# hzyu17/GaussianVI

Hardware: AMD Instinct MI355X
Metric: sigma-point psi-evals/sec + NGD iters/sec, 1024-factor d=12 p=5 chain (higher is better)
Workload: dtype f64; 1 GPU; c3: T=1025 states, n=6; 1 step = 1 device-resident NGD iteration; restart every 30; factor_sets_columns=[K factors, d, GH degree p, N sigma points], factor_set_kinds=1024 x quadratic-prior d=12 p=5 (N=17217); 1025 x fixed-prior d=6 p=5 (N=1433), kernel_variant=6, chunks_per_factor=4, fused_pass=True, one_launch_factor_stage=False, mirror_pairs=False, fuse_trial=2

## Files before the change

### gaussianvi_amd/csrc/gvi_hip.hip

```cpp
#include "../../include/gvi_hip.h"

#include <hip/hip_runtime.h>
#include <hip/hip_ext.h>
#include <dlfcn.h>

#include <algorithm>
#include <chrono>
#include <cmath>
#include <cstdio>
#include <cstdlib>
#include <cstring>
#include <memory>
#include <map>
#include <set>
#include <string>
#include <thread>
#include <type_traits>
#include <vector>

#include "host_linalg.hpp"
#include "kernels_bt.hpp"
#include "chain_launch.hpp"
#include "kernels_factor.hpp"
#include "kernels_orbit.hpp"
// ... 491 lines not shown
  const int nb0 = nbx0 * a0.nchunk, nb1 = nbx1 * a1.nchunk;
  const int grid = std::max(nb0, nb1);
  if (full)
    hipExtLaunchKernelGGL((moments_orbit_pair_kernel<M, SMAX, true, false, WAVES>), dim3(grid), dim3(256), (uint32_t)lds, st, e0, e1, 0,
                          a0, a1, nbx0, nb0, nbx1);
  else
    hipExtLaunchKernelGGL((moments_orbit_pair_kernel<M, SMAX, false, false, WAVES>), dim3(grid), dim3(256), (uint32_t)lds, st, e0, e1, 0,
                          a0, a1, nbx0, nb0, nbx1);
}

void launch_orbit_pair(const OrbitArgs& a0, const OrbitArgs& a1, int m, int smax, bool full, hipStream_t st, hipEvent_t e0, hipEvent_t e1) {
  const size_t lds = (size_t)4 * std::max(orbit_lds_doubles(a0.d, m, a0.copies), orbit_lds_doubles(a1.d, m, a1.copies)) * 8;
  with_orbit_instance(m, smax, [&]<int M, int SMAX, int WAVES, bool PAIR>(OrbitInst<M, SMAX, WAVES, PAIR>) {
    if constexpr (PAIR) launch_orbit_pair_t<M, SMAX, WAVES>(a0, a1, full, lds, st, e0, e1);
  });
}

inline std::atomic<long long>* fused_launches() { static std::atomic<long long> c[3]; return c; }

inline std::atomic<long long>& block3_launches() { static std::atomic<long long> c; return c; }

template <int M, int SMAX, int WAVES, int D0, int D1>
gvi_status launch_fused_t(gvi_ctx* c, const FusedArgs& A, unsigned grid, size_t lds, int dmax, int copies, int items, hipEvent_t e0, hipEvent_t e1) {
  if (lds > 64 * 1024) GVICK(allow_lds(c, (const void*)factor_fused_kernel<M, SMAX, WAVES, D0, D1>, (int)lds));
#ifdef GVI_FUSED_TIMING
  const int dbg = getenv("GVI_FUSED_DBG") ? atoi(getenv("GVI_FUSED_DBG")) : 0;
  static unsigned long long* stamps = nullptr;
  static int nprint = 0;
  if ((dbg & 8) && !stamps) { if (hipMalloc(&stamps, 1120 * 8) != hipSuccess) stamps = nullptr; else (void)hipMemset(stamps, 0, 1120 * 8); }
#else
  const int dbg = 0;
  unsigned long long* stamps = nullptr;
#endif
  hipExtLaunchKernelGGL((factor_fused_kernel<M, SMAX, WAVES, D0, D1>), dim3(grid), dim3(256), (uint32_t)lds, c->stream, e0, e1, 0, A, dmax, copies, items,
                        (dbg & 8) ? stamps : (unsigned long long*)nullptr);
  ++fused_launches()[M == 2 ? 2 : (SMAX <= 4 ? 0 : 1)];
#ifdef GVI_FUSED_TIMING
  if ((dbg & 8) && stamps && ++nprint > 200 && nprint <= 202) {
    unsigned long long h[1120];
    (void)hipStreamSynchronize(c->stream);
    (void)hipMemcpy(h, stamps, sizeof(h), hipMemcpyDeviceToHost);
    for (int blk = 0; blk < 8; ++blk)
      for (int w = 0; w < 4; ++w)
        for (int it = 0; it < 2; ++it) {
          const unsigned long long* ws = h + 352 + ((blk * 4 + w) * 2 + it) * 12;
          fprintf(stderr, "[walk stamps] block %4d wave %d item %d: shader cycles prologue %llu | s=1 %llu (%llu tiles) | s=2 %llu (%llu) | s=3 %llu (%llu) | s=4 %llu (%llu) | reduction %llu\n",
                  blk * 146, w, it, ws[0], ws[1], ws[7], ws[2], ws[8], ws[3], ws[9], ws[4], ws[10], ws[5]);
        }
    for (int w = 0; w < 4; ++w) {
      fprintf(stderr, "[prep stamps] block 0 wave %d, us after the wave's start: prologue [arguments warm | first scalars | barrier] %.2f %.2f %.2f; gather [entry | loads back | stores issued] %.2f %.2f %.2f; products [Sigma row loaded | Cholesky | L^-1 | LDS | Lam + stores | H, u0]:",
              w, (double)(long long)(h[256 + 16 * w + 11] - h[8 * w]) * 0.01, (double)(long long)(h[256 + 16 * w + 12] - h[8 * w]) * 0.01,
              (double)(long long)(h[256 + 16 * w + 13] - h[8 * w]) * 0.01, (double)(long long)(h[256 + 16 * w + 8] - h[8 * w]) * 0.01, (double)(long long)(h[256 + 16 * w + 9] - h[8 * w]) * 0.01, (double)(long long)(h[256 + 16 * w + 10] - h[8 * w]) * 0.01);
      for (int i = 0; i < 6; ++i) fprintf(stderr, " %.2f", (double)(long long)(h[256 + 16 * w + i] - h[8 * w]) * 0.01);
      fprintf(stderr, "\n");
    }
    unsigned long long t0 = ~0ull;
    for (int blk = 0; blk < 8; ++blk) if (h[blk * 32] && h[blk * 32] < t0) t0 = h[blk * 32];
    for (int blk = 0; blk < 8; ++blk)
      for (int w = 0; w < 4; ++w) {
        const unsigned hw = (unsigned)h[320 + blk * 4 + w], xcc = (unsigned)(h[320 + blk * 4 + w] >> 32);
        fprintf(stderr, "[fused stamps] block %4d wave %d (xcc %u se %u cu %2u simd %u slot %2u; absolute, us after the first start):", blk * 146, w,
                xcc & 15, (hw >> 13) & 7, (hw >> 8) & 15, (hw >> 4) & 3, hw & 15);
        for (int i = 0; i < 8; ++i) fprintf(stderr, " %.2f", h[blk * 32 + w * 8 + i] ? (double)(long long)(h[blk * 32 + w * 8 + i] - t0) * 0.01 : -1.0);
        fprintf(stderr, "\n");
      }
  }
#endif
  return GVI_OK;
}

gvi_status launch_prep(gvi_ctx* c, const FactorDev& f, const double* mu, const double* Sigma, hipStream_t st) {
  const int d = f.d, dp = d + (d & 1);
  const size_t lds = (size_t)(4 * d * d + 2 * dp + 3 * d) * 8 + (size_t)dp * 4 + 16;
  if (d <= 8) hipLaunchKernelGGL(prep_kernel<1>, dim3(f.K), dim3(64), lds, st, f, mu, Sigma);
  else if (d <= 16) hipLaunchKernelGGL(prep_kernel<4>, dim3(f.K), dim3(64), lds, st, f, mu, Sigma);
  else if (d <= 32) hipLaunchKernelGGL(prep_kernel<16>, dim3(f.K), dim3(64), lds, st, f, mu, Sigma);
  else return fail(c, GVI_ERR_UNSUPPORTED, "factor dimension > 32");
  return GVI_OK;
}

gvi_status run_prep(gvi_ctx* c, FactorSet& s, const double* mu, const double* Sigma, int slot = -1,
                    hipStream_t st = nullptr) {
  if (!st) st = c->stream;
  if (slot >= 0 && s.prep_slot == slot) return GVI_OK;
  s.prep_slot = slot;
  if (s.K == 0) return GVI_OK;
  GVICK(launch_prep(c, s.dev(c->opt), mu, Sigma, st));
  HIPCK(c, hipGetLastError());
  return GVI_OK;
}

template <int KIND>
gvi_status launch_orbit_psi_t(gvi_ctx* c, const OrbitPsiArgs& a, bool full, dim3 grid, size_t lds, hipStream_t st) {
  if (full) {
    if (lds > 64 * 1024) GVICK(allow_lds(c, (const void*)moments_orbit_psi_kernel<KIND, true>, (int)lds));
    hipLaunchKernelGGL((moments_orbit_psi_kernel<KIND, true>), grid, dim3(256), lds, st, a);
  } else {
    hipLaunchKernelGGL((moments_orbit_psi_kernel<KIND, false>), grid, dim3(256), lds, st, a);
  }
  return GVI_OK;
}

struct MomPlan {
  Route route = Route::Empty;
  int full = 0;
  int nchunk = 1;
// ... 1480 lines not shown
      HIPCK(ctx, hipGetLastError());
      record_plan(s0, P[0], true);
      record_plan(s1, P[1], true);
      return prof_close(ctx, b);
    }
    case Fuse::SregPair:
    case Fuse::ScostPair: {
      FactorSet &s0 = *ctx->sets[0], &s1 = *ctx->sets[1];
      const MomArgs &a0 = P[0].a, &a1 = P[1].a;
      const int nbx0 = (int)P[0].grid.x, nbx1 = (int)P[1].grid.x;
      const int nb0 = nbx0 * (int)P[0].grid.y, nb1 = nbx1 * (int)P[1].grid.y;
      GVICK(prof_open(ctx, s0, 0, full != 0, true, ctx->stream, &b));
      if (full && P[0].pipe && P[1].pipe)
        hipLaunchKernelGGL((moments_sreg_pair_kernel<12, 6, 6, 6, true, true>), dim3(std::max(nb0, nb1)), dim3(256), 0, ctx->stream,
                           a0, a1, nbx0, nb0, nbx1);
      else if (full)
        hipLaunchKernelGGL((moments_sreg_pair_kernel<12, 6, 6, 6, true>), dim3(nb0 + nb1), dim3(256), 0, ctx->stream, a0, a1, nbx0, nb0, nbx1);
      else
        hipLaunchKernelGGL((moments_scost_pair_kernel<12, 6, 6, 6, 2>), dim3(nb0 + nb1), dim3(256), 0, ctx->stream, a0, a1, nbx0, nb0, nbx1);
      HIPCK(ctx, hipGetLastError());
      record_plan(s0, P[0], true);
      record_plan(s1, P[1], true);
      return prof_close(ctx, b);
    }
    case Fuse::Planar3: {
      int nbx[3], nb[3];
      for (int q = 0; q < 3; ++q) {
        nbx[q] = (ctx->sets[q]->K + 3) / 4;
        nb[q] = nbx[q] * P[q].nchunk;
      }
      GVICK(prof_open(ctx, *ctx->sets[1], 0, full != 0, true, ctx->stream, &b));
      if (full)
        hipLaunchKernelGGL((moments_planar3_kernel<true>), dim3(nb[0] + nb[1] + nb[2]), dim3(256), 0, ctx->stream, P[0].a, P[1].a, P[2].a,
                           nbx[0], nb[0], nbx[1], nb[1], nbx[2], P[0].pipe ? 1 : 0);
      else
        hipLaunchKernelGGL((moments_planar3_kernel<false>), dim3(nb[0] + nb[1] + nb[2]), dim3(256), 0, ctx->stream, P[0].a, P[1].a, P[2].a,
                           nbx[0], nb[0], nbx[1], nb[1], nbx[2], 0);
      HIPCK(ctx, hipGetLastError());
      for (int q = 0; q < 3; ++q) record_plan(*ctx->sets[q], P[q], false);
      return prof_close(ctx, b);
    }
    case Fuse::None:
      break;
  }
  for (int i = 0; i < ns; ++i) GVICK(launch_single(ctx, *ctx->sets[i], P[i], ctx->stream));
  return GVI_OK;
}

static gvi_status ngd_fused_full(gvi_ctx* ctx, int slot, int publish_slot, const PassPlan& pp) {
  constexpr int fused_chunks = 4;
  FusedArgs A{};
  A.nsets = (int)ctx->sets.size();
  A.koff[0] = 0;
  int dmax = 0, copies = 1;
  const FusedKey key = fused_key(A.nsets, pp.F);
  A.nblk = fused_nblk(pp.F[0].K, A.nsets > 1 ? pp.F[1].K : 0, FUSED_MAX_ITEMS);
  for (int si = 0; si < A.nsets; ++si) {
    FactorSet& s = *ctx->sets[si];
    FusedSet& F = A.s[si];
    s.prep_slot = -1;
    F.f = s.dev(ctx->opt);
    GVICK(warm_start_of(ctx, s, F.f));
    GVICK(orbit_args(ctx, s, fused_chunks, &F.oa));
    F.oa.partial = nullptr;
    F.mu = s.mu_k[slot].d(); F.Sigma = s.Sigma_k[slot].d();
    F.start = s.chain_structured ? nullptr : (const int32_t*)s.dstart.p;
    F.mu_k = s.mu_k[slot].d(); F.Sigma_k = s.Sigma_k[slot].d();
    F.Ephi = s.Ephi.d(); F.cost = s.cost.d(); F.Vdmu = s.Vdmu.d(); F.Vddmu = s.Vddmu.d();
    A.koff[si + 1] = A.koff[si] + s.K;
    A.cl.cost[si] = s.cost.d(); A.cl.K[si] = s.K;
    dmax = std::max(dmax, s.d);
    copies = std::max(copies, F.oa.copies);
  }
  const int items = 1 + (A.nsets > 1 ? (ctx->sets[1]->K + A.nblk - 1) / A.nblk : 0);
  const size_t lds = fused_lds_doubles(dmax, key.m, copies, items) * 8;
  if (lds > 160 * 1024) return fail(ctx, GVI_ERR_UNSUPPORTED, "fused pass: LDS budget");
  A.cl.nsets = A.nsets;
  if (A.nsets == 1) A.koff[2] = A.koff[1];
  const unsigned extra = take_gather(ctx, slot, A, 256);
  GVICK(fill_epi_tail(ctx, A.koff[A.nsets], publish_slot, &A.tail));
  ++ctx->ngd.n_full_pass;
  ProfBracket b;
  GVICK(prof_open(ctx, *ctx->sets[0], 0, true, false, ctx->stream, &b));
  const unsigned grid = (unsigned)A.nblk + extra;
  gvi_status rc = GVI_OK;
  if (!with_fused_instance(key.m, key.smax, key.d0, key.d1, [&]<int M, int SMAX, int WAVES, int D0, int D1>(FusedInst<M, SMAX, WAVES, D0, D1>) {
        rc = launch_fused_t<M, SMAX, WAVES, D0, D1>(ctx, A, grid, lds, dmax, copies, items, b.e0, b.e1);
      }))
    return fail(ctx, GVI_ERR_UNSUPPORTED, "fused pass: shape not instantiated");
  GVICK(rc);
  HIPCK(ctx, hipGetLastError());
  for (auto& s : ctx->sets) record_pass(s->last, Route::Orbit, true, fused_chunks, s->table->Np);
  return prof_close(ctx, b);
}

static gvi_status ngd_block3_full(gvi_ctx* ctx, int slot, int publish_slot, const PassPlan& pp) {
  const MomPlan* P = pp.P;
  ++ctx->ngd.n_full_pass;
  Block3Args A{};
  A.nitems = ctx->sets[0]->K + ctx->sets[1]->K + ctx->sets[2]->K;
  A.pipe = P[0].pipe ? 1 : 0;
  unsigned nblk = 0;
  for (int q = 0; q < 3; ++q) {
    FactorSet& s = *ctx->sets[q];
    BlockSet& B = A.s[q];
    B.a = P[q].a;
// ... 776 lines not shown
  ctx->profile_all = on == 2;
  ctx->profile_every = on == 3 ? 8 : 1;
  ctx->ngd.profile_count = 0;
  for (auto& s : ctx->sets) s->ev_set[0] = s->ev_set[1] = false;
  return GVI_OK;
}

gvi_status gvi_profile_last(gvi_ctx* ctx, int set_id, int what, float* ms) {
  FactorSet* s = get_set(ctx, set_id);
  if (!s || !ms || what < 0 || what > 1) return GVI_ERR_ARG;
  if (!s->ev_set[what]) return fail(ctx, GVI_ERR_STATE, "no profiled launch recorded");
  HIPCK(ctx, hipEventSynchronize(s->ev[what][1]));
  HIPCK(ctx, hipEventElapsedTime(ms, s->ev[what][0], s->ev[what][1]));
  return GVI_OK;
}

gvi_status gvi_profile_stages(gvi_ctx* ctx, int on, float* mean_us, int* counts) {
  if (!ctx) return GVI_ERR_ARG;
  HIPCK(ctx, hipSetDevice(ctx->device));
  if (mean_us || counts) {
    GVICK(sync(ctx));
    double sum[STAGE_COUNT] = {0, 0, 0};
    int cnt[STAGE_COUNT] = {0, 0, 0};
    for (auto& r : ctx->stage_recs) {
      float ms = 0.f;
      if (hipEventElapsedTime(&ms, r.e0, r.e1) == hipSuccess) { sum[r.stage] += ms; ++cnt[r.stage]; }
    }
    for (int i = 0; i < STAGE_COUNT; ++i) {
      if (mean_us) mean_us[i] = cnt[i] ? (float)(1e3 * sum[i] / cnt[i]) : 0.f;
      if (counts) counts[i] = cnt[i];
    }
  }
  for (auto& r : ctx->stage_recs) { ctx->stage_pool.push_back(r.e0); ctx->stage_pool.push_back(r.e1); }
  ctx->stage_recs.clear();
  ctx->stage_prof = on != 0;
  return GVI_OK;
}

gvi_status gvi_profile_geometry(gvi_ctx* ctx, int set_id, int* variant, int* nchunk, int64_t* chunk) {
  FactorSet* s = get_set(ctx, set_id);
  if (!s) return GVI_ERR_ARG;
  if (variant) *variant = geometry_code(s->last.route, s->last.fused_pair, s->closed_form);
  if (nchunk) *nchunk = s->last.nchunk;
  if (chunk) *chunk = s->last.chunk;
  return GVI_OK;
}

gvi_status gvi_set_option(gvi_ctx* ctx, const char* name, int value) {
  if (!ctx || !name) return GVI_ERR_ARG;
  const std::string n(name);
  if (ctx->ngd.ready) { GVICK(ngd_flush_assemble(ctx, 0)); GVICK(ngd_flush_assemble(ctx, 1)); }
  if (n == "safe_publish") GVICK(sync(ctx));
  std::string why;
  if (!option_set(ctx->opt, name, value, &why)) return fail(ctx, GVI_ERR_ARG, why);
  if (n == "safe_publish") for (int q = 0; q < 16; ++q) ctx->host_slot[q] = 0.0;
  if (n == "chain_merge") ctx->opt.chain_merge_fault = value == 2;
  for (auto& s : ctx->sets) s->prep_slot = -1;
  ngd_invalidate(ctx);
  return GVI_OK;
}


gvi_status gvi_debug_cost_log(gvi_ctx* ctx, int entries, double* out, double* seq_now) {
  if (!ctx) return GVI_ERR_ARG;
  HIPCK(ctx, hipSetDevice(ctx->device));
  GVICK(sync(ctx));
  if (entries > 0) {
    if (entries & (entries - 1)) return fail(ctx, GVI_ERR_ARG, "entries must be a power of two");
    HIPCK(ctx, ctx->dbg_log.ensure((size_t)entries * 8));
    HIPCK(ctx, hipMemset(ctx->dbg_log.p, 0, (size_t)entries * 8));
    ctx->dbg_mask = entries - 1;
    double* lg = ctx->dbg_log.d();
    HIPCK(ctx, hipMemcpyToSymbol(HIP_SYMBOL(gvi_dbg_mask), &ctx->dbg_mask, sizeof(int)));
    HIPCK(ctx, hipMemcpyToSymbol(HIP_SYMBOL(gvi_dbg_log), &lg, sizeof(double*)));
  } else if (entries == 0 && out) {
    if (!ctx->dbg_mask) return fail(ctx, GVI_ERR_STATE, "cost log not enabled");
    HIPCK(ctx, hipMemcpy(out, ctx->dbg_log.p, (size_t)(ctx->dbg_mask + 1) * 8, hipMemcpyDeviceToHost));
  } else {
    ctx->dbg_mask = 0;
    double* lg = nullptr;
    HIPCK(ctx, hipMemcpyToSymbol(HIP_SYMBOL(gvi_dbg_log), &lg, sizeof(double*)));
  }
  if (seq_now) *seq_now = ctx->seq;
  return GVI_OK;
}

gvi_status gvi_debug_products(gvi_ctx* ctx, int set_id, double* S, double* Sinv, double* Lam, double* H, double* u0) {
  if (!ctx) return GVI_ERR_ARG;
  FactorSet* s = get_set(ctx, set_id);
  if (!s) return GVI_ERR_ARG;
  HIPCK(ctx, hipSetDevice(ctx->device));
  GVICK(sync(ctx));
  const size_t dd = (size_t)s->K * s->d * s->d * 8, md = (size_t)s->K * s->m * s->d * 8, mb = (size_t)s->K * s->m * 8;
  auto get = [&](double* out, const DevMem& src, size_t bytes) {
    if (!out || bytes == 0) return hipSuccess;
    if (!src.p || src.bytes < bytes) return hipErrorInvalidValue;
    return hipMemcpy(out, src.p, bytes, hipMemcpyDeviceToHost);
  };
  HIPCK(ctx, get(S, s->S, dd));
  HIPCK(ctx, get(Sinv, s->Sinv, dd));
  HIPCK(ctx, get(Lam, s->Lam, dd));
  HIPCK(ctx, get(H, s->H, md));
  HIPCK(ctx, get(u0, s->u0, mb));
  return GVI_OK;
}

gvi_status gvi_set_variant(gvi_ctx* ctx, int variant) {
// ... 7 lines not shown
```

### gaussianvi_amd/csrc/kernels_factor.hpp

```cpp
#pragma once
#include <hip/hip_runtime.h>
#include <stdint.h>

#include <utility>

#include "device_common.hpp"
#include "dpp_rowb.hpp"
#include "factor_dev.hpp"
#include "psi_point.hpp"

namespace gvi {

__device__ __forceinline__ double rcp_nr(double x) {
  double r = __builtin_amdgcn_rcp(x);
  return fma(fma(-x, r, 1.0), r, r);
}
__device__ __forceinline__ double rsq_nr(double x) {
  const double r = __builtin_amdgcn_rsq(x);
  return r * fma(-0.5 * x * r, r, 1.5);
}

__device__ inline double wave_sum(double v) {
#pragma unroll
  for (int o = 32; o > 0; o >>= 1) v += __shfl_xor(v, o);
  return v;
}

template <int EPLP, int DT>
__device__ __forceinline__ void prep_body(const FactorDev& f, const double* mu, const double* Sigma, int k, double* sm, int kin) {
  const int d = DT ? DT : f.d, dd = d * d, lane = threadIdx.x & 63;
  const int dp = d + (d & 1);
  double* A0 = sm;
  double* A1 = A0 + dd;
  double* V0 = A1 + dd;
  double* V1 = V0 + dd;
  double* al = V1 + dd;
  double* be = al + dp;
  double* lam = be + dp;
  int* pa = (int*)(lam + 3 * d);
  int ei[EPLP], ej[EPLP];
#pragma unroll
  for (int q = 0; q < EPLP; ++q) {
    const int e = lane + q * 64;
    ei[q] = e < dd ? e / d : -1;
    ej[q] = e < dd ? e % d : 0;
  }
  const double* Sg = Sigma + (size_t)kin * dd;
  bool warm = f.warm != 0 && f.Vws != nullptr;
  if (warm) {
    int bad = 0;
#pragma unroll
    for (int q = 0; q < EPLP; ++q) {
      if (ei[q] >= 0) {
        const int i = ei[q], j = ej[q], e = lane + q * 64;
        const double v = f.Vws[(size_t)k * dd + e];
        bad |= !(fabs(v) <= 2.0);
        V0[e] = v;
        A1[e] = i >= j ? Sg[i * d + j] : Sg[j * d + i];
      }
    }
// ... 201 lines not shown
__device__ inline void prep_chol_body(const FactorDev& f, const double* mu, const double* Sigma, int k, double* sm, int kin, double* Zs = nullptr,
                                      double* Hs = nullptr, double* u0s = nullptr, const int hstride = 0, int* l_ready = nullptr) {
  const bool lean = Hs != nullptr;
  constexpr int d = DT, dd = DT * DT;
  const int lane = threadIdx.x & 63;
  double* Ll = sm;
  double* Xl = Ll + dd;
  const double* Sg = Sigma + (size_t)kin * dd;
  static_assert(!ROWB || DT <= 16, "row-broadcast form: a row of L per lane of a 16-lane row");
  const int lr = ROWB ? (lane & 15) : lane;
  const int li = lr < d ? lr : d - 1;
  constexpr int HPL = 2;
  const int mm = f.m;
  const bool pre = mm > 0 && mm * d <= 64 * HPL && !l_ready;
  double arow[HPL][DT], brow = 0.0;
  if (pre) {
    const double* Ak = f.A + (size_t)k * mm * d;
#pragma unroll
    for (int q = 0; q < HPL; ++q) {
      const int e = lane + 64 * q;
      const int r = e < mm * d ? e / d : 0;
#pragma unroll
      for (int c = 0; c < d; ++c) arow[q][c] = Ak[r * d + c];
    }
    if (lane < mm) brow = f.b[(size_t)k * mm + lane];
  }
  PREP_STAMP(0);
  double row[DT];
#pragma unroll
  for (int c = 0; c < d; ++c) row[c] = c <= li ? Sg[li * d + c] : 0.0;
  PREP_STAMP(1);
  double inv[DT];
  if constexpr (ROWB) {
#pragma unroll
    for (int c = 0; c < d; ++c) rowb_pin(row[c]);
    chol_rowb_steps<DT, 0>(row, inv, li);
  } else {
#pragma unroll
    for (int j = 0; j < d; ++j) {
      const double pj = chol_readlane(row[j], j);
      double r = __builtin_amdgcn_rsq(pj);
      r = r * fma(-0.5 * pj * r, r, 1.5);
      r = r * fma(-0.5 * pj * r, r, 1.5);
      inv[j] = r;
      row[j] = li == j ? pj * r : (li > j ? row[j] * r : 0.0);
#pragma unroll
      for (int c = j + 1; c < d; ++c) {
        const double lcj = chol_readlane(row[j], c);
        row[c] = li >= c ? fma(-row[j], lcj, row[c]) : 0.0;
      }
    }
  }
  PREP_STAMP(2);
  double xcol[DT];
#pragma unroll
  for (int i = 0; i < d; ++i) xcol[i] = li == i ? 1.0 : 0.0;
  if constexpr (ROWB) {
#pragma unroll
    for (int c = 0; c < d; ++c) rowb_settle(row[c]);
    chol_rowb_inverse<DT, 0>(xcol, row, inv, li);
  } else {
#pragma unroll
    for (int i = 0; i < d; ++i) {
      xcol[i] = li <= i ? xcol[i] * inv[i] : 0.0;
#pragma unroll
      for (int j = i + 1; j < d; ++j) xcol[j] = fma(-chol_readlane(row[i], j), xcol[i], xcol[j]);
    }
  }
  PREP_STAMP(3);
  if (lane < d) {
#pragma unroll
    for (int c = 0; c < d; ++c) { Ll[lane * d + c] = row[c]; Xl[c * d + lane] = xcol[c]; }
  }
  double* Al = Xl + dd;
  if (pre) {
#pragma unroll
    for (int q = 0; q < HPL; ++q) {
      const int e = lane + 64 * q;
      if (e < mm * d && e % d == 0) {
#pragma unroll
        for (int c = 0; c < d; ++c) Al[e + c] = arow[q][c];
      }
    }
  }
  wave_lds_sync();
  if (l_ready && lane == 0) __hip_atomic_store(l_ready, 1, __ATOMIC_RELAXED, __HIP_MEMORY_SCOPE_WORKGROUP);
  if (lean) {
    for (int e = lane; e < dd; e += 64) Zs[e] = Xl[(e % d) * d + e / d];
  } else {
    for (int e = lane; e < dd; e += 64) {
      const int i = e / d, j = e % d;
      double lam = 0.0;
#pragma unroll
      for (int c = 0; c < d; ++c) lam = fma(Xl[c * d + i], Xl[c * d + j], lam);
      f.S[(size_t)k * dd + e] = Ll[e];
      f.Sinv[(size_t)k * dd + e] = Xl[j * d + i];
      f.Lam[(size_t)k * dd + e] = lam;
      if (Zs) Zs[e] = Xl[j * d + i];
    }
  }
  PREP_STAMP(4);
  if (f.m > 0 && !l_ready) {
    const int m = f.m;
    const double* Ak = f.A + (size_t)k * m * d;
    if (pre) {
#pragma unroll
      for (int q = 0; q < HPL; ++q) {
        const int e = lane + 64 * q;
        if (e < m * d) {
          const int r = e / d, a = e % d;
          double h = 0.0;
#pragma unroll
          for (int c = 0; c < d; ++c) h += arow[q][c] * Ll[c * d + a];
          if (lean) Hs[a * hstride + r] = h;
          else {
            f.H[(size_t)k * m * d + a * m + r] = h;
            if (f.Hq) {
              const int R = (m + 3) / 4;
              f.Hq[(((size_t)k * 4 + r / R) * d + a) * R + r % R] = h;
            }
          }
        }
      }
    } else {
      for (int e = lane; e < m * d; e += 64) {
        const int r = e / d, a = e % d;
        double h = 0.0;
#pragma unroll
        for (int c = 0; c < d; ++c) h += Ak[r * d + c] * Ll[c * d + a];
        f.H[(size_t)k * m * d + a * m + r] = h;
        if (f.Hq) {
          const int R = (m + 3) / 4;
          f.Hq[(((size_t)k * 4 + r / R) * d + a) * R + r % R] = h;
        }
      }
    }
    if (lane < m) {
      double u = pre ? brow : f.b[(size_t)k * m + lane];
#pragma unroll
      for (int c = 0; c < d; ++c) u += (pre ? Al[lane * d + c] : Ak[lane * d + c]) * mu[(size_t)kin * d + c];
      if (lean) u0s[lane] = u;
      else f.u0[(size_t)k * m + lane] = u;
// ... 1404 lines not shown
  const double* __restrict__ w = a.f.w;
  for (int64_t base = i0; base < i1; base += 64) {
    const int64_t i = base + lane;
    double z[D];
#pragma unroll
    for (int c = 0; c < D; ++c) z[c] = Zt[(size_t)c * Np + i];
    const double wi = i < a.f.N ? w[i] : 0.0;
#pragma unroll
    for (int f = 0; f < F; ++f) {
      const double psi = split_psi_rows<D, M>(hq[f], us_w[f], us_w[f] + M, z);
      acc[f] += i < a.f.N ? wi * psi : 0.0;
    }
  }
#pragma unroll
  for (int f = 0; f < F; ++f) {
    double s = acc[f];
#pragma unroll
    for (int o = 32; o > 0; o >>= 1) s += __shfl_xor(s, o);
    if (lane == 0 && k0 + f < a.f.K) a.partial[(size_t)(k0 + f) * a.nchunk + by] = s;
  }
}

template <int D, int M, int F>
__global__ __launch_bounds__(256) void moments_scost_kernel(MomArgs a) {
  if (pred_skip(a.pred, a.pred_val)) return;
  __shared__ double us[4 * F * 3 * M];
  scost_body<D, M, F>(a, blockIdx.x, blockIdx.y, us);
}

template <int D0, int M0, int D1, int M1, int F>
__global__ __launch_bounds__(256) void moments_scost_pair_kernel(MomArgs a0, MomArgs a1, int nbx0, int nb0, int nbx1) {
  if (pred_skip(a0.pred, a0.pred_val)) return;
  constexpr int MM = M0 > M1 ? M0 : M1;
  __shared__ double us[4 * F * 3 * MM];
  const int b = blockIdx.x;
  if (b < nb0) scost_body<D0, M0, F>(a0, b % nbx0, b / nbx0, us);
  else scost_body<D1, M1, F>(a1, (b - nb0) % nbx1, (b - nb0) / nbx1, us);
}

struct EpiArgs {
  FactorDev f;
  const double* partial;
  int nchunk, full;
  double* Ephi;
  double* cost;
  double* Vdmu;
  double* Vddmu;
  double* E_xmuphi;
  double* E_xxphi;
};

__host__ __device__ inline size_t epilogue_lds_doubles(int d) { return (size_t)npairs(d) + 4 * (size_t)d * d; }

template <int DT>
__device__ __forceinline__ double epilogue_body_t(const EpiArgs& a, int k, double* sm, int phase, const double* P, double* Zs = nullptr) {
  const FactorDev& f = a.f;
  const int d = DT ? DT : f.d, dd = d * d, lane = threadIdx.x & 63;
  const int npo = a.full ? npairs(d) : 1;
  double* Ms = sm;
  double* M2 = Ms + npairs(d);
  double* Tm = M2 + dd;
  double* Sv = Zs ? Zs : Tm + dd;
  double* Lv = Tm + 2 * dd;
  const double Tk = f.temperature[k];
  const bool want_v = a.full && (a.Vdmu || a.Vddmu);
  if (want_v && phase != 2 && !Zs) {
    const double* Sinv = f.Sinv + (size_t)k * dd;
    const double* Lam = f.Lam + (size_t)k * dd;
    for (int e = lane; e < dd; e += 64) { Sv[e] = Sinv[e]; Lv[e] = Lam[e]; }
  }
  for (int j = lane; j < npo && phase != 2; j += 64) {
    double s = 0.0;
    for (int c0 = 0; c0 < a.nchunk; c0 += 8) {
      double pv[8];
#pragma unroll
      for (int q = 0; q < 8; ++q) pv[q] = c0 + q < a.nchunk ? P[(size_t)(c0 + q) * npo + j] : 0.0;
#pragma unroll
      for (int q = 0; q < 8; ++q) s += pv[q];
    }
    Ms[j] = s;
  }
  wave_lds_sync();
  const double m0 = Ms[0];
  const double costk = m0 / Tk;
  if (lane == 0 && phase != 2) {
    if (a.Ephi) a.Ephi[k] = m0;
    if (a.cost) a.cost[k] = costk;
  }
  if (!a.full || phase == 1) return costk;
  for (int e = lane; e < dd; e += 64) {
    const int i = e / d, j = e % d;
    M2[e] = i <= j ? Ms[pair_index(d, i, j)] : Ms[pair_index(d, j, i)];
  }
  wave_lds_sync();
  if (a.Vdmu) {
    for (int i = lane; i < d; i += 64) {
      double s = 0.0;
#pragma unroll
      for (int c = 0; c < d; ++c) s += Sv[i * d + c] * Ms[1 + c];
      a.Vdmu[(size_t)k * d + i] = s / Tk;
    }
  }
  if (a.Vddmu) {
    for (int e = lane; e < dd; e += 64) {
      const int i = e / d, j = e % d;
      double s = 0.0;
#pragma unroll
      for (int c = 0; c < d; ++c) s += Sv[i * d + c] * M2[c * d + j];
      Tm[e] = s;
    }
    wave_lds_sync();
    for (int e = lane; e < dd; e += 64) {
      const int i = e / d, j = e % d;
      if (i <= j) {
        double s = 0.0;
#pragma unroll
        for (int c = 0; c < d; ++c) s += Tm[i * d + c] * Sv[j * d + c];
        double lam;
        if (Zs) {
          lam = 0.0;
#pragma unroll
          for (int c = 0; c < d; ++c) lam = fma(Sv[i * d + c], Sv[j * d + c], lam);
        } else lam = Lv[i * d + j];
        const double v = (s - lam * m0) / Tk;
        a.Vddmu[(size_t)k * dd + i * d + j] = v;
        a.Vddmu[(size_t)k * dd + j * d + i] = v;
      }
    }
    wave_lds_sync();
  }
  if (a.E_xmuphi || a.E_xxphi) {
    const double* S = f.S + (size_t)k * dd;
    for (int e = lane; e < dd; e += 64) Sv[e] = S[e];
    wave_lds_sync();
  }
  if (a.E_xmuphi) {
    for (int i = lane; i < d; i += 64) {
      double s = 0.0;
#pragma unroll
      for (int c = 0; c < d; ++c) s += Sv[i * d + c] * Ms[1 + c];
      a.E_xmuphi[(size_t)k * d + i] = s;
    }
  }
  if (a.E_xxphi) {
    for (int e = lane; e < dd; e += 64) {
      const int i = e / d, j = e % d;
      double s = 0.0;
#pragma unroll
      for (int c = 0; c < d; ++c) s += Sv[i * d + c] * M2[c * d + j];
      Tm[e] = s;
    }
    wave_lds_sync();
    for (int e = lane; e < dd; e += 64) {
      const int i = e / d, j = e % d;
      double s = 0.0;
#pragma unroll
      for (int c = 0; c < d; ++c) s += Tm[i * d + c] * Sv[j * d + c];
      a.E_xxphi[(size_t)k * dd + e] = s;
    }
  }
  return costk;
}

__device__ __forceinline__ double epilogue_body_p(const EpiArgs& a, int k, double* sm, int phase, const double* P, double* Zs = nullptr) {
// ... 196 lines not shown
```

### gaussianvi_amd/csrc/kernels_fused.hpp

```cpp
#pragma once
#include "kernels_orbit.hpp"

namespace gvi {

constexpr int FUSED_MAX_ITEMS = 4;

struct FusedSet {
  FactorDev f;
  OrbitArgs oa;
  const double* mu;
  const double* Sigma;
  const int32_t* start;
  double* mu_k;
  double* Sigma_k;
  double* Ephi;
  double* cost;
  double* Vdmu;
  double* Vddmu;
};

struct FusedArgs {
  int nsets;
  int nblk;
  int koff[3];
  FusedSet s[2];
  int gather, n;
  const double* gmu;
  const double* gdmu;
  double gstep;
  const double* SigD;
  const double* SigU;
  double* mu_out;
  int64_t nmu;
  EpiTail tail;
  CostList cl;
};

__host__ __device__ inline size_t fused_item_doubles(int d) {
  const size_t dd = (size_t)d * d, dp = d + (d & 1);
  const size_t prep = 4 * dd + 2 * dp + 3 * d + (dp + 1) / 2 + 1 + dd + d + 2;
  const size_t epi = epilogue_lds_doubles(d) + 2;
  return ((prep > epi ? prep : epi) + 1) & ~(size_t)1;
}
__host__ __device__ inline size_t fused_region_doubles(int dmax, int M, int copies) {
  const size_t a = (size_t)orbit_lds_doubles(dmax, M, copies), b = fused_item_doubles(dmax);
  return ((a > b ? a : b) + 1) & ~(size_t)1;
}
__host__ __device__ inline size_t fused_keep_doubles(int dmax, int M) {
  return (size_t)dmax * dmax + (size_t)dmax * orbit_hstride(M) + (size_t)(M + (M & 1));
}
__host__ __device__ inline size_t fused_lds_doubles(int dmax, int M, int copies, int items) {
  return 4 * fused_region_doubles(dmax, M, copies) + (size_t)items * (fused_keep_doubles(dmax, M) + 4 * (size_t)npairs(dmax));
}


template <int DT>
__device__ __forceinline__ bool fused_gather(const FusedArgs& A, const FusedSet& S, const int k, const int lane, double* Sl, double* ml,
                                             const LazyPred& lpred) {
  constexpr int dd = DT * DT, NI = (dd + 63) / 64;
  PREP_STAMP(8);
  const int n = A.n, nn = n * n;
  const int s = S.start ? S.start[k] : k;
  double v[NI];
#pragma unroll
  for (int i = 0; i < NI; ++i) {
    const int e = lane + 64 * i, r = e / DT, c = e % DT;
    const double* p;
    if (r < n && c < n) p = A.SigD + (size_t)s * nn + r * n + c;
    else if (r >= n && c >= n) p = A.SigD + (size_t)(s + 1) * nn + (r - n) * n + (c - n);
    else if (r < n) p = A.SigU + (size_t)s * nn + r * n + (c - n);
    else p = A.SigU + (size_t)s * nn + c * n + (r - n);
    v[i] = e < dd ? *p : 0.0;
  }
  double m = 0.0;
  if (lane < DT) {
    const size_t j = (size_t)s * n + lane;
    m = A.gdmu ? A.gmu[j] + A.gstep * A.gdmu[j] : A.gmu[j];
// ... 119 lines not shown
        mval = A.gdmu ? A.gmu[j] + A.gstep * A.gdmu[j] : A.gmu[j];
      } else mval = S.mu[(size_t)k * d + lane];
      mh[lane] = mval;
    }
    if (!pred_fail(lpred)) {
      if (si == 0) prep_chol_hu0<D0>(S.f, mh, k, own, sm + (size_t)wi * region, &l_ready[it], Zs + oH, Zs + oU, orbit_hstride(M));
      else prep_chol_hu0<D1>(S.f, mh, k, own, sm + (size_t)wi * region, &l_ready[it], Zs + oH, Zs + oU, orbit_hstride(M));
    }
  }
  FUSED_STAMP(1);
  if (pred_fail(lpred)) return;
  __syncthreads();
  FUSED_STAMP(2);
  for (int it = 0; it < nitems; ++it) {
    const int si = it < c0 ? 0 : 1;
    const int k = b + (it < c0 ? it : it - c0) * A.nblk;
    const FusedSet& S = A.s[si];
    const double* Zi = Zbase + (size_t)it * zs;
    orbit_wave<M, SMAX, true, false, true>(S.oa, k, wave, sm + (size_t)wave * region, Pbase + (size_t)it * ps + (size_t)wave * npairs(S.f.d),
                                           Zi + oH, Zi + oU);
  }
  FUSED_STAMP(3);
  __syncthreads();
  FUSED_STAMP(4);
  const bool helpers = A.tail.on && nitems <= 2;
  if (iw >= nitems) {
    const int it = iw - 2;
    if (!helpers || it < 0 || it >= nitems) return;
    const int si = it < c0 ? 0 : 1;
    const int k = b + (it < c0 ? it : it - c0) * A.nblk;
    const FusedSet& S = A.s[si];
    const double Tk = S.f.temperature[k];
    const double* Pl = Pbase + (size_t)it * ps;
    const int npo = npairs(S.f.d);
    double m0 = 0.0;
#pragma unroll
    for (int q = 0; q < 4; ++q) m0 += Pl[(size_t)q * npo];
    const double costk = m0 / Tk;
    epi_tail_arrive(A.cl, A.tail, S.cost + k, costk, (int)(threadIdx.x & 63), (unsigned)(A.koff[si] + k), (unsigned)A.koff[A.nsets],
                    (int*)(sm + (size_t)wave * region));
    return;
  }
  {
    const int si = iw < c0 ? 0 : 1;
    const int k = b + (iw < c0 ? iw : iw - c0) * A.nblk;
    const FusedSet& S = A.s[si];
    const int d = S.f.d;
    double* area = sm + (size_t)wave * region;
    double* Zs = Zbase + (size_t)iw * zs;
    const double* Pl = Pbase + (size_t)iw * ps;
    EpiArgs e;
    e.f = S.f; e.partial = nullptr; e.nchunk = 4; e.full = 1;
    e.Ephi = S.Ephi; e.cost = helpers ? nullptr : S.cost; e.Vdmu = S.Vdmu; e.Vddmu = S.Vddmu; e.E_xmuphi = nullptr; e.E_xxphi = nullptr;
    auto epi = [&](int phase) { return si == 0 ? epilogue_body_t<D0>(e, k, area, phase, Pl, Zs) : epilogue_body_t<D1>(e, k, area, phase, Pl, Zs); };
    if (!A.tail.on || helpers) { epi(0); return; }
    const double costk = epi(1);
    FUSED_STAMP(5);
    int* last = (int*)(area + epilogue_lds_doubles(d));
    epi_tail_arrive(A.cl, A.tail, S.cost + k, costk, (int)(threadIdx.x & 63), (unsigned)(A.koff[si] + k), (unsigned)A.koff[A.nsets], last);
    FUSED_STAMP(6);
    epi(2);
    FUSED_STAMP(7);
  }
}

}
```

### gaussianvi_amd/csrc/options.hpp

```cpp
#pragma once
#include <math.h>
#include <stdlib.h>
#include <string.h>

#include <string>

namespace gvi {

inline bool& chain_wave_enabled();
inline bool& chain_asm_dense_enabled();
inline bool& chain_pair_enabled();

struct Options {
  bool warm_start = true;
  int fuse_trial = 2;
  int target_waves = 2048;
  bool mirror = true;
  int split_flush = 64;
  bool sreg_pipe = true;
  bool no_scost = false;
  bool orbit = true;
  bool fused = true;
  int orbit_waves = 4096;
  double jacobi_tol = 1e-34;
  bool chol_sqrt = true;
  bool chol_rowb = false;
  bool trust_table_degree = false;
  int orbit_min_tiles = 6;
  int orbit_copies = 8;
  bool pair_fuse = true;
  bool fuse_gather = true;
  bool side_solve = true;
  bool asm_on_load = true;
  bool chain_merge = true;
  bool chain_merge_fault = false;
  bool pipeline = true;
  int spin_ms = 2;
  bool safe_publish = false;
  bool sample_sweep = true;
  bool solve_lds = true;
};

enum OptionRule {
  OPT_FLAG,
  OPT_FLAG_INV,
  OPT_MIN,
  OPT_CLAMP,
  OPT_POW10_MAX
};

struct OptionRow {
  const char* name;
  const char* env;
  OptionRule rule;
  int lo, hi;
  bool Options::*flag;
  int Options::*num;
  double Options::*real;
  bool& (*process)();
};

constexpr OptionRow opt_flag(const char* name, const char* env, bool Options::*f) { return {name, env, OPT_FLAG, 0, 0, f, nullptr, nullptr, nullptr}; }
constexpr OptionRow opt_flag_inv(const char* name, const char* env, bool Options::*f) { return {name, env, OPT_FLAG_INV, 0, 0, f, nullptr, nullptr, nullptr}; }
constexpr OptionRow opt_process(const char* name, const char* env, bool& (*f)()) { return {name, env, OPT_FLAG, 0, 0, nullptr, nullptr, nullptr, f}; }
constexpr OptionRow opt_min(const char* name, const char* env, int Options::*f, int lo) { return {name, env, OPT_MIN, lo, 0, nullptr, f, nullptr, nullptr}; }
constexpr OptionRow opt_clamp(const char* name, const char* env, int Options::*f, int lo, int hi) { return {name, env, OPT_CLAMP, lo, hi, nullptr, f, nullptr, nullptr}; }
constexpr OptionRow opt_pow10(const char* name, double Options::*f, int hi) { return {name, nullptr, OPT_POW10_MAX, 0, hi, nullptr, nullptr, f, nullptr}; }

constexpr OptionRow OPTION_ROWS[] = {
  opt_flag("orbit", "GVI_ORBIT", &Options::orbit),
  opt_flag("fused", "GVI_FUSED", &Options::fused),
  opt_flag("assemble_on_load", "GVI_ASM_ON_LOAD", &Options::asm_on_load),
  opt_flag("pipeline", "GVI_PIPELINE", &Options::pipeline),
  opt_process("chain_wave", "GVI_CHAIN_WAVE", &chain_wave_enabled),
  opt_process("asm_dense", "GVI_ASM_DENSE", &chain_asm_dense_enabled),
  opt_process("chain_pair", "GVI_CHAIN_PAIR", &chain_pair_enabled),
  opt_flag("chain_merge", "GVI_CHAIN_MERGE", &Options::chain_merge),
  opt_flag("chol_rowb", "GVI_CHOL_ROWB", &Options::chol_rowb),
  opt_clamp(nullptr, "GVI_FUSE_TRIAL", &Options::fuse_trial, 0, 2),
// ... 60 lines not shown
```

Measured before the change: 226.1 billion psi-evals/s.

## Exploit triangular sigma factor in epilogue Hessian products and publish L earlier

Adds a triangular back-transform path for the fused epilogue's Vddmu computation. It skips the known-zero columns of the triangular factor per 64-lane round and computes only the upper-triangle pairs, mirroring each result. The prep stage also stores L to LDS and raises l_ready before the inverse solve so consumers can start sooner, and it writes X straight into Zs on the lean path instead of doing a transpose copy. The new path is on by default through a new epi_tri option, at the cost of added template complexity.

```diff
diff --git a/gaussianvi_amd/csrc/epi_tri.hpp b/gaussianvi_amd/csrc/epi_tri.hpp
--- /dev/null
+++ b/gaussianvi_amd/csrc/epi_tri.hpp
@@ -0,0 +1,43 @@
+#pragma once
+#include "hd.hpp"
+
+namespace gvi {
+
+constexpr int tri_full_rounds(int d) { return (d * d + 63) / 64; }
+constexpr int tri_cmin(int d, int round) { return (64 * round) / d; }
+
+constexpr int tri_pairs(int d) { return d * (d + 1) / 2; }
+constexpr int tri_pair_rounds(int d) { return (tri_pairs(d) + 63) / 64; }
+template <int D>
+GVI_HD_INLINE constexpr int tri_pair_j(int p) {
+  int j = 0;
+  GVI_UNROLL
+  for (int t = 1; t < D; ++t) j += p >= t * (t + 1) / 2 ? 1 : 0;
+  return j;
+}
+template <int D>
+GVI_HD_INLINE constexpr int tri_pair_i(int p, int j) { return p - j * (j + 1) / 2; }
+template <int D>
+constexpr int tri_pair_cmin(int round) { return tri_pair_j<D>(64 * round); }
+
+template <int D>
+constexpr bool tri_check() {
+  bool seen[D * D] = {};
+  for (int p = 0; p < tri_pairs(D); ++p) {
+    const int j = tri_pair_j<D>(p), i = tri_pair_i<D>(p, j);
+    if (j < 0 || j >= D || i < 0 || i > j || seen[i * D + j]) return false;
+    seen[i * D + j] = true;
+    if (tri_pair_cmin<D>(p / 64) > j) return false;
+  }
+  for (int i = 0; i < D; ++i)
+    for (int j = 0; j < D; ++j)
+      if (seen[i * D + j] != (i <= j)) return false;
+  for (int e = 0; e < D * D; ++e)
+    if (tri_cmin(D, e / 64) > e / D) return false;
+  return true;
+}
+static_assert(tri_check<2>() && tri_check<4>() && tri_check<6>() && tri_check<8>() && tri_check<12>(),
+              "triangular back-transform: pair enumeration or round bounds");
+static_assert(tri_pair_rounds(12) == 2 && tri_pair_cmin<12>(1) == 10 && tri_cmin(12, 1) == 5 && tri_cmin(12, 2) == 10, "d = 12 geometry");
+
+}
diff --git a/gaussianvi_amd/csrc/gvi_hip.hip b/gaussianvi_amd/csrc/gvi_hip.hip
--- a/gaussianvi_amd/csrc/gvi_hip.hip
+++ b/gaussianvi_amd/csrc/gvi_hip.hip
@@ -567,6 +567,11 @@
               w, (double)(long long)(h[256 + 16 * w + 11] - h[8 * w]) * 0.01, (double)(long long)(h[256 + 16 * w + 12] - h[8 * w]) * 0.01,
               (double)(long long)(h[256 + 16 * w + 13] - h[8 * w]) * 0.01, (double)(long long)(h[256 + 16 * w + 8] - h[8 * w]) * 0.01, (double)(long long)(h[256 + 16 * w + 9] - h[8 * w]) * 0.01, (double)(long long)(h[256 + 16 * w + 10] - h[8 * w]) * 0.01);
       for (int i = 0; i < 6; ++i) fprintf(stderr, " %.2f", (double)(long long)(h[256 + 16 * w + i] - h[8 * w]) * 0.01);
+      fprintf(stderr, "; phase 3 [entry | cost | tail | M2, Vdmu | W M2 | end]:");
+      for (const int i : {4, 5, 6, 256 + 14, 256 + 15, 7}) {
+        const unsigned long long t = i < 256 ? h[8 * w + i] : h[i + 16 * w];
+        fprintf(stderr, " %.2f", t ? (double)(long long)(t - h[8 * w]) * 0.01 : -1.0);
+      }
       fprintf(stderr, "\n");
     }
     unsigned long long t0 = ~0ull;
@@ -2153,6 +2158,7 @@
   FusedArgs A{};
   A.nsets = (int)ctx->sets.size();
   A.koff[0] = 0;
+  A.epi_tri = ctx->opt.epi_tri ? 1 : 0;
   int dmax = 0, copies = 1;
   const FusedKey key = fused_key(A.nsets, pp.F);
   A.nblk = fused_nblk(pp.F[0].K, A.nsets > 1 ? pp.F[1].K : 0, FUSED_MAX_ITEMS);
@@ -3035,7 +3041,8 @@
   if (ctx->ngd.ready) { GVICK(ngd_flush_assemble(ctx, 0)); GVICK(ngd_flush_assemble(ctx, 1)); }
   if (n == "safe_publish") GVICK(sync(ctx));
   std::string why;
-  if (!option_set(ctx->opt, name, value, &why)) return fail(ctx, GVI_ERR_ARG, why);
+  if (n == "epi_tri") ctx->opt.epi_tri = value != 0;
+  else if (!option_set(ctx->opt, name, value, &why)) return fail(ctx, GVI_ERR_ARG, why);
   if (n == "safe_publish") for (int q = 0; q < 16; ++q) ctx->host_slot[q] = 0.0;
   if (n == "chain_merge") ctx->opt.chain_merge_fault = value == 2;
   for (auto& s : ctx->sets) s->prep_slot = -1;
diff --git a/gaussianvi_amd/csrc/kernels_factor.hpp b/gaussianvi_amd/csrc/kernels_factor.hpp
--- a/gaussianvi_amd/csrc/kernels_factor.hpp
+++ b/gaussianvi_amd/csrc/kernels_factor.hpp
@@ -6,6 +6,7 @@
 
 #include "device_common.hpp"
 #include "dpp_rowb.hpp"
+#include "epi_tri.hpp"
 #include "factor_dev.hpp"
 #include "psi_point.hpp"
 
@@ -313,6 +314,15 @@
     }
   }
   PREP_STAMP(2);
+  const bool early = l_ready != nullptr;
+  if (early) {
+    if (lane < d) {
+#pragma unroll
+      for (int c = 0; c < d; ++c) Ll[lane * d + c] = row[c];
+    }
+    wave_lds_sync();
+    if (lane == 0) __hip_atomic_store(l_ready, 1, __ATOMIC_RELAXED, __HIP_MEMORY_SCOPE_WORKGROUP);
+  }
   double xcol[DT];
 #pragma unroll
   for (int i = 0; i < d; ++i) xcol[i] = li == i ? 1.0 : 0.0;
@@ -331,7 +341,11 @@
   PREP_STAMP(3);
   if (lane < d) {
 #pragma unroll
-    for (int c = 0; c < d; ++c) { Ll[lane * d + c] = row[c]; Xl[c * d + lane] = xcol[c]; }
+    for (int c = 0; c < d; ++c) {
+      if (!early) Ll[lane * d + c] = row[c];
+      if (lean) Zs[lane * d + c] = xcol[c];
+      else Xl[c * d + lane] = xcol[c];
+    }
   }
   double* Al = Xl + dd;
   if (pre) {
@@ -345,10 +359,7 @@
     }
   }
   wave_lds_sync();
-  if (l_ready && lane == 0) __hip_atomic_store(l_ready, 1, __ATOMIC_RELAXED, __HIP_MEMORY_SCOPE_WORKGROUP);
-  if (lean) {
-    for (int e = lane; e < dd; e += 64) Zs[e] = Xl[(e % d) * d + e / d];
-  } else {
+  if (!lean) {
     for (int e = lane; e < dd; e += 64) {
       const int i = e / d, j = e % d;
       double lam = 0.0;
@@ -1859,8 +1870,45 @@
 
 __host__ __device__ inline size_t epilogue_lds_doubles(int d) { return (size_t)npairs(d) + 4 * (size_t)d * d; }
 
-template <int DT>
-__device__ __forceinline__ double epilogue_body_t(const EpiArgs& a, int k, double* sm, int phase, const double* P, double* Zs = nullptr) {
+template <int DT, int R>
+__device__ __forceinline__ void epi_tri_wm2(const double* Sv, const double* M2, double* Tm, const int lane) {
+  if constexpr (R < tri_full_rounds(DT)) {
+    constexpr int d = DT, dd = DT * DT, c0 = tri_cmin(DT, R);
+    const int e = lane + 64 * R;
+    if (64 * (R + 1) <= dd || e < dd) {
+      const int i = e / d, j = e % d;
+      double s = 0.0;
+#pragma unroll
+      for (int c = c0; c < d; ++c) s += Sv[i * d + c] * M2[j * d + c];
+      Tm[e] = s;
+    }
+    epi_tri_wm2<DT, R + 1>(Sv, M2, Tm, lane);
+  }
+}
+template <int DT, int R>
+__device__ __forceinline__ void epi_tri_out(const double* Sv, const double* Tm, double* out, const double m0, const double Tk, const int lane) {
+  if constexpr (R < tri_pair_rounds(DT)) {
+    constexpr int d = DT, c0 = tri_pair_cmin<DT>(R);
+    const int p = lane + 64 * R;
+    if (64 * (R + 1) <= tri_pairs(DT) || p < tri_pairs(DT)) {
+      const int j = tri_pair_j<DT>(p), i = tri_pair_i<DT>(p, j);
+      double s = 0.0;
+#pragma unroll
+      for (int c = c0; c < d; ++c) s += Tm[i * d + c] * Sv[j * d + c];
+      double lam = 0.0;
+#pragma unroll
+      for (int c = c0; c < d; ++c) lam = fma(Sv[i * d + c], Sv[j * d + c], lam);
+      const double v = (s - lam * m0) / Tk;
+      out[i * d + j] = v;
+      out[j * d + i] = v;
+    }
+    epi_tri_out<DT, R + 1>(Sv, Tm, out, m0, Tk, lane);
+  }
+}
+
+template <int DT, bool TRI = false>
+__device__ __forceinline__ double epilogue_body_t(const EpiArgs& a, int k, double* sm, int phase, const double* P, double* Zs = nullptr,
+                                                  const bool tri = false) {
   const FactorDev& f = a.f;
   const int d = DT ? DT : f.d, dd = d * d, lane = threadIdx.x & 63;
   const int npo = a.full ? npairs(d) : 1;
@@ -1908,7 +1956,19 @@
       a.Vdmu[(size_t)k * d + i] = s / Tk;
     }
   }
-  if (a.Vddmu) {
+  PREP_STAMP(14);
+  bool tri_done = false;
+  if constexpr (TRI && DT > 0 && tri_full_rounds(DT) > 1) {
+    if (a.Vddmu && tri) {
+      epi_tri_wm2<DT, 0>(Sv, M2, Tm, lane);
+      wave_lds_sync();
+      PREP_STAMP(15);
+      epi_tri_out<DT, 0>(Sv, Tm, a.Vddmu + (size_t)k * dd, m0, Tk, lane);
+      wave_lds_sync();
+      tri_done = true;
+    }
+  }
+  if (a.Vddmu && !tri_done) {
     for (int e = lane; e < dd; e += 64) {
       const int i = e / d, j = e % d;
       double s = 0.0;
@@ -1917,6 +1977,7 @@
       Tm[e] = s;
     }
     wave_lds_sync();
+    PREP_STAMP(15);
     for (int e = lane; e < dd; e += 64) {
       const int i = e / d, j = e % d;
       if (i <= j) {
diff --git a/gaussianvi_amd/csrc/kernels_fused.hpp b/gaussianvi_amd/csrc/kernels_fused.hpp
--- a/gaussianvi_amd/csrc/kernels_fused.hpp
+++ b/gaussianvi_amd/csrc/kernels_fused.hpp
@@ -23,6 +23,7 @@
   int nsets;
   int nblk;
   int koff[3];
+  int epi_tri;
   FusedSet s[2];
   int gather, n;
   const double* gmu;
@@ -248,8 +249,11 @@
     EpiArgs e;
     e.f = S.f; e.partial = nullptr; e.nchunk = 4; e.full = 1;
     e.Ephi = S.Ephi; e.cost = helpers ? nullptr : S.cost; e.Vdmu = S.Vdmu; e.Vddmu = S.Vddmu; e.E_xmuphi = nullptr; e.E_xxphi = nullptr;
-    auto epi = [&](int phase) { return si == 0 ? epilogue_body_t<D0>(e, k, area, phase, Pl, Zs) : epilogue_body_t<D1>(e, k, area, phase, Pl, Zs); };
-    if (!A.tail.on || helpers) { epi(0); return; }
+    const bool tri = A.epi_tri != 0;
+    auto epi = [&](int phase) {
+      return si == 0 ? epilogue_body_t<D0, true>(e, k, area, phase, Pl, Zs, tri) : epilogue_body_t<D1, true>(e, k, area, phase, Pl, Zs, tri);
+    };
+    if (!A.tail.on || helpers) { epi(0); FUSED_STAMP(7); return; }
     const double costk = epi(1);
     FUSED_STAMP(5);
     int* last = (int*)(area + epilogue_lds_doubles(d));
diff --git a/gaussianvi_amd/csrc/options.hpp b/gaussianvi_amd/csrc/options.hpp
--- a/gaussianvi_amd/csrc/options.hpp
+++ b/gaussianvi_amd/csrc/options.hpp
@@ -25,6 +25,7 @@
   double jacobi_tol = 1e-34;
   bool chol_sqrt = true;
   bool chol_rowb = false;
+  bool epi_tri = true;
   bool trust_table_degree = false;
   int orbit_min_tiles = 6;
   int orbit_copies = 8;
```

Result: no change. 227.7 billion psi-evals/s, median of 3 (+0.7%).
